# knights-lab/UTree

Measured on AMD Instinct MI355X. Metric: reads classified/sec, 8 GB L2 CTR, 150 bp reads, higher is better.
Workload: dtype u64

## Files before the change

utree_amd/csrc/dev_image.c:

```c
#define _FILE_OFFSET_BITS 64
#define _GNU_SOURCE
#define __HIP_PLATFORM_AMD__ 1
#include <hip/hip_runtime_api.h>
#include <fcntl.h>
#include <math.h>
#include <stddef.h>
#include <stdio.h>
#include <stdlib.h>
#include <string.h>
#include <unistd.h>
#include "ctr_host.h"
#include "dev_image.h"

#define HIPCHK(x) do { hipError_t e_ = (x); if (e_ != hipSuccess) { utree_dev_set_hip_error((int)e_, #x); rc = e_ == hipErrorOutOfMemory ? UTREE_E_NOMEM : UTREE_E_HIP; goto fail; } } while (0)
#define KCHK(x) do { int e_ = (x); if (e_ != 0) { utree_dev_set_hip_error(e_, #x); rc = e_ == (int)hipErrorOutOfMemory ? UTREE_E_NOMEM : UTREE_E_HIP; goto fail; } } while (0)

static __thread char g_hip_msg[256];
void utree_dev_set_hip_error(int err, const char *what) {
    snprintf(g_hip_msg, sizeof g_hip_msg, "%s (%d) in %s", hipGetErrorString((hipError_t)err), err, what);
    if (getenv("UTREE_DEBUG")) fprintf(stderr, "[utree_amd] HIP error: %s\n", g_hip_msg);
}
const char *utree_last_hip_error(void) { return g_hip_msg; }

#include <time.h>
// ... 123 lines not shown
    }
    h->off_coarse = off; off = align_up(off + (uint64_t)UTREE_NUMBINS * ((h->flags & UTREE_F_OFF64) ? 8 : 4), 256);
    h->off_irreg = off; off = align_up(off + (1u << 24) / 8, 256);
    h->off_label_off = off; off = align_up(off + ((uint64_t)h->n_labels + 1) * 4, 256);
    uint64_t blob = 0;
    for (uint32_t i = 0; i < h->n_labels; ++i) blob += (uint64_t)ctr->label_len[i] + 1;
    h->label_blob_bytes = blob;
    h->off_label_blob = off; off = align_up(off + blob + 64, 256);
    h->off_rank2ix = off; off = align_up(off + (uint64_t)h->n_labels * 4, 256);
    h->off_vote = off; off = align_up(off + (uint64_t)h->n_labels * sizeof(utk_vote_rec), 4096);
    h->off_recs = off; off = align_up(off + (h->n_nodes + 8) * h->rec_words * 8, 4096);
    h->total_bytes = off;
}

size_t utree_dev_image_bytes(const utree_ctr *ctr, int fine_bits) {
    if (!ctr) return 0;
    utree_image_header h;
    layout(ctr, (uint32_t)utree_pick_fine_bits(ctr, fine_bits), &h);
    return (size_t)h.total_bytes;
}

static void bind_image(utree_dev *d) {
    char *b = (char *)d->image;
    d->kimg.table = (const uint64_t *)(b + d->hdr.off_table);
    d->kimg.regions = (const uint64_t *)(b + offsetof(utree_image_header, regions));
    d->kimg.mrecs = (const uint64_t *)(b + d->hdr.off_mrecs);
    d->kimg.recs = (const uint64_t *)(b + d->hdr.off_recs);
    d->kimg.coarse = b + d->hdr.off_coarse;
    d->kimg.irreg = (const uint32_t *)(b + d->hdr.off_irreg);
    d->kimg.label_off = (const uint32_t *)(b + d->hdr.off_label_off);
    d->kimg.label_blob = b + d->hdr.off_label_blob;
    d->kimg.rank2ix = (const uint32_t *)(b + d->hdr.off_rank2ix);
    d->kimg.vote_tab = (d->hdr.flags & UTREE_F_VOTE_TABLE) && !getenv("UTREE_VOTE_BYTES") ? (const uint64_t *)(b + d->hdr.off_vote) : NULL;
    d->kimg.n_nodes = d->hdr.n_nodes;
    d->kimg.n_labels = d->hdr.n_labels;
    d->kimg.fine_bits = d->hdr.fine_bits;
    d->kimg.flags = d->hdr.flags;
    d->kimg.W = d->hdr.W; d->kimg.I = d->hdr.I;
    d->kimg.bucket_words = d->hdr.bucket_words;
    {
        const char *e = getenv("UTREE_OVF_SCAN");
        d->kimg.ovf_scan = e && atoi(e) > 0 && atoi(e) <= 1024 ? (uint32_t)atoi(e) : (d->hdr.n_min * 4 > d->hdr.n_nodes ? 16u : 32u);
    }
    d->kimg.irr_n = 0;
    for (int i = 0; i < 4; ++i) d->kimg.irr_p[i] = 0xFFFFFFFFu;
    if (d->hdr.flags & UTREE_F_GENERIC) d->kimg.irr_n = 0xFFFFFFFFu;
    else if (d->hdr.flags & UTREE_F_IRREGULAR) {
        d->kimg.irr_n = 0xFFFFFFFFu;
        uint32_t *bm = d->hdr.n_irregular <= 4 ? (uint32_t *)malloc((1u << 24) / 8) : NULL;
        if (bm && hipMemcpy(bm, d->kimg.irreg, (1u << 24) / 8, hipMemcpyDeviceToHost) == hipSuccess) {
            uint32_t n = 0, p[4] = {0, 0, 0, 0};
            for (uint32_t w = 0; w < (1u << 24) / 32 && n <= 4; ++w)
                for (uint32_t x = bm[w]; x && n <= 4; x &= x - 1) { if (n < 4) p[n] = w * 32 + (uint32_t)__builtin_ctz(x); ++n; }
            if (n <= 4) { d->kimg.irr_n = n; for (uint32_t i = 0; i < n; ++i) d->kimg.irr_p[i] = p[i]; }
        } else (void)hipGetLastError();
        free(bm);
    }
}

static void lanes_ring_init(utree_dev *d);
static int device_ok(int device, int *n_cu) {
    int n = 0;
    if (hipGetDeviceCount(&n) != hipSuccess || device < 0 || device >= n) return UTREE_E_HIP;
    if (hipSetDevice(device) != hipSuccess) return UTREE_E_HIP;
    hipDeviceProp_t p;
    if (hipGetDeviceProperties(&p, device) != hipSuccess) return UTREE_E_HIP;
// ... 613 lines not shown
        if (w.long_blocks) {
            if (e0) HIPCHK(hipEventRecord(e0, st));
            HIPCHK(hipMemsetAsync(w.ltab_rank, 0xFF, (size_t)w.n_long_cap * UTREE_LONG_SLOTS * 4, st));
            HIPCHK(hipMemsetAsync(w.ltab_cnt, 0, (size_t)w.n_long_cap * UTREE_LONG_SLOTS * 4, st));
            HIPCHK(hipMemsetAsync(w.lflag, 0, (size_t)w.n_long_cap * 4, st));
            KCHK(utk_classify_long_pieces(&d->kimg, d_bases, d_off, d_len, do_rc, d_out, &w, d->n_cu, st));
            utk_workspace wl = w;
            wl.long_list = w.long_left;
            wl.long_blocks = w.long_blocks >= 8 ? w.long_blocks / 8 : 1;
            KCHK(utk_classify_long(&d->kimg, d_bases, d_off, d_len, do_rc, d_out, &wl, d->n_cu, st));
            if (e0) { HIPCHK(hipEventRecord(e1, st)); d->recorded[tslot] = 1; }
        }
        KCHK(utk_classify_listed(&d->kimg, d_bases, d_off, d_len, n_reads, max_len, do_rc, d_out, &w, d->n_cu, st));
        if (e0 && !w.long_blocks) { HIPCHK(hipEventRecord(e1, st)); d->recorded[tslot] = 1; }
    } else {
        const int dominant = w.long_blocks ? 2 : (w.mid_reads ? 1 : 0);
        d->last_long = dominant == 2; d->last_mid = dominant == 1; d->last_rc = do_rc; d->last_short_cap = w.short_cap;
        d->last_lanes = 0; d->last_mixed = 0; d->last_pieces = 0;
        if (w.mid_reads) KCHK(utk_route(d_len, n_reads, do_rc, &w, st));
        if (e0 && dominant == 0) HIPCHK(hipEventRecord(e0, st));
        KCHK(utk_classify_short(&d->kimg, d_bases, d_off, d_len, n_reads, do_rc, d_out, &w, d->n_cu, st));
        if (e0 && dominant == 0) { HIPCHK(hipEventRecord(e1, st)); d->recorded[tslot] = 1; }
        if (w.mid_reads) {
            if (e0 && dominant == 1) HIPCHK(hipEventRecord(e0, st));
            KCHK(utk_classify_mid(&d->kimg, d_bases, d_off, d_len, n_reads, do_rc, d_out, &w, d->n_cu, st));
            if (e0 && dominant == 1) { HIPCHK(hipEventRecord(e1, st)); d->recorded[tslot] = 1; }
        }
        if (w.long_blocks) {
            if (e0) HIPCHK(hipEventRecord(e0, st));
            KCHK(utk_classify_long(&d->kimg, d_bases, d_off, d_len, do_rc, d_out, &w, d->n_cu, st));
            if (e0) { HIPCHK(hipEventRecord(e1, st)); d->recorded[tslot] = 1; }
        }
    }
    KCHK(utk_vote(&d->kimg, d_out, &w, n_reads, st));
    if (ring_post(d, &w, lanes ? n_reads : 0, st)) { (void)hipGetLastError(); }
    { ring_lock(d); const unsigned long long pe = d->dev_error; ring_unlock(d);
      if (pe) { rc = UTREE_E_DEVICE; snprintf(g_hip_msg, sizeof g_hip_msg, "an earlier batch's kernels reported error %llu: utree_classify_poll returns (and clears) it", pe); } }
#ifdef UTREE_LANES_TIMERS
    { extern void utk_lanes_phase_dump(void); static int lcalls; if (++lcalls == 6) utk_lanes_phase_dump(); }
#endif
#ifdef UTREE_PHASE_TIMERS
    { extern void utk_phase_dump(void); static int calls; if (++calls == 12) utk_phase_dump(); }
#endif
fail:
    return rc;
}

int utree_lookup_words(utree_dev *d, const uint64_t *d_hi, const uint64_t *d_lo, uint64_t n, uint32_t *d_ix, void *stream) {
    int rc = UTREE_OK;
    if (!d || !d_lo || !d_ix) return UTREE_E_ARG;
    if (d->hdr.W == 16 && !d_hi) return UTREE_E_ARG;
    HIPCHK(hipSetDevice(d->device));
    KCHK(utk_lookup(&d->kimg, d_hi, d_lo, n, d_ix, (hipStream_t)stream));
fail:
    return rc;
}

const char *utree_classify_kernel_name(const utree_dev *dc) {
    if (!dc) return "";
    utree_dev *d = (utree_dev *)dc;
    if (d->last_lanes && d->last_pieces) {
        snprintf(d->kernel_sig, sizeof d->kernel_sig, "classify_lanes_k<%u, %u, 16, %s, 2, %u, %s>", d->hdr.W, d->hdr.I, d->kimg.irr_n ? "true" : "false", d->hdr.bucket_words / 8,
                 utk_lanes_both_strands(&d->kimg, d->last_rc) ? "true" : "false");
        return d->kernel_sig;
    }
    if (d->last_lanes && d->last_mixed) {
        snprintf(d->kernel_sig, sizeof d->kernel_sig, "classify_lanes_mixed_k<%u, %u, %s, %u, %s>", d->hdr.W, d->hdr.I, d->kimg.irr_n ? "true" : "false",
// ... 53 lines not shown
```

utree_amd/csrc/kernels.hip:

```cpp
#include <hip/hip_runtime.h>
#include <stdint.h>
#include <stdio.h>
#include <string.h>
#include "device_common.hpp"
#include "wave_common.hpp"

using namespace utk;

namespace {

#ifdef UTREE_PHASE_TIMERS
__device__ unsigned long long g_phase[16];
struct PhaseT { unsigned long long t, acc[12]; };
#define PH_DECL PhaseT ph_; ph_.t = __builtin_readcyclecounter(); for (int q_ = 0; q_ < 12; ++q_) ph_.acc[q_] = 0;
#define TICKP(ph, i) do { const unsigned long long n_ = __builtin_readcyclecounter(); (ph).acc[i] += n_ - (ph).t; (ph).t = n_; } while (0)
#define TICK(i) TICKP(ph_, i)
#define PH_ARG , PhaseT &ph_
#define PH_PASS , ph_
#define PH_WAITVM asm volatile("s_waitcnt vmcnt(0)" ::: "memory")
#else
#define PH_DECL
#define TICK(i)
#define PH_ARG
#define PH_PASS
#define PH_WAITVM
#endif


constexpr uint32_t KEY_TILE = 128;

struct LaneBits {
    const uint32_t *swl;
    uint32_t sh;
};
__device__ __forceinline__ LaneBits lane_bits(const uint32_t *sw, uint32_t lane) {
    LaneBits b;
    const uint32_t r = lane & 15u;
    b.swl = sw + (lane >> 4) - (r == 0 ? 1u : 0u);
// ... 612 lines not shown
#pragma unroll
        for (int d = 1; d < 64; d <<= 1) { uint32_t t = __shfl_up(inc, d); if (lane >= (uint32_t)d) inc += t; }
        if (lane == 63) s_scan[wv] = inc;
        __syncthreads();
        uint32_t wbase = 0, uix = 0;
        for (uint32_t w = 0; w < LONG_THREADS / 64; ++w) { if (w < wv) wbase += s_scan[w]; uix += s_scan[w]; }
        uint32_t pos = wbase + inc - cnt;
        if (tid == 0) s_base = uix > 1 ? reserve_tally(ws, (unsigned long long)uix) : 0ull;
        __syncthreads();
        const unsigned long long base = s_base;
        for (uint32_t x = lo; x < hi; ++x) {
            uint32_t bits = __hip_atomic_load(&touch[x], __ATOMIC_RELAXED, __HIP_MEMORY_SCOPE_AGENT);
            if (!bits) continue;
            __hip_atomic_store(&touch[x], 0u, __ATOMIC_RELAXED, __HIP_MEMORY_SCOPE_AGENT);
            while (bits) {
                const uint32_t rk = x * 32 + (uint32_t)__builtin_ctz(bits);
                bits &= bits - 1;
                const uint32_t c = __hip_atomic_load(&hist[rk], __ATOMIC_RELAXED, __HIP_MEMORY_SCOPE_AGENT);
                __hip_atomic_store(&hist[rk], 0u, __ATOMIC_RELAXED, __HIP_MEMORY_SCOPE_AGENT);
                if (uix > 1) ws.tally[base + pos] = (uint64_t)rk | ((uint64_t)c << 32);
                else s_single = rk;
                ++pos;
            }
        }
        __syncthreads();
        if (tid == 0) {
            if (uix == 1) store_result(&out[r], im.rank2ix[s_single], -2, F, 1, 0, 0);
            else store_result(&out[r], 0, CUT_PENDING, F, uix, (uint32_t)base, (uint32_t)(base >> 32));
        }
        __syncthreads();
    }
}

__device__ __forceinline__ uint32_t cut_of(uint32_t x) {
    uint32_t c = x - x / 4;
    c += (x >> 1) >= c;
    return c;
}

__device__ __forceinline__ void label16(const char *s, uint32_t p, uint64_t &x, uint64_t &y) {
    typedef unsigned long long u64x2 __attribute__((ext_vector_type(2), aligned(1)));
    const u64x2 v = *(const u64x2 *)(s + p);
    x = v.x; y = v.y;
}

__device__ __forceinline__ uint64_t stop_flags(uint64_t x1, uint64_t x2) {
    const uint64_t semi = x1 ^ 0x3B3B3B3B3B3B3B3Bull, d = x1 ^ x2;
    uint64_t m = (((x1 - 0x0101010101010101ull) & ~x1) | ((semi - 0x0101010101010101ull) & ~semi)) & 0x8080808080808080ull;
    m |= (((d & 0x7F7F7F7F7F7F7F7Full) + 0x7F7F7F7F7F7F7F7Full) | d) & 0x8080808080808080ull;
    return m;
}

__device__ __forceinline__ void pair_scan(const char *s1, const char *s2, uint32_t start, uint32_t &td, uint32_t &a, uint32_t &b, uint32_t &before) {
    uint32_t base = start, prevlast = start ? (uint32_t)(uint8_t)s1[start - 1] : 0u;
    for (;;) {
        uint64_t x1, y1, x2, y2;
        label16(s1, base, x1, y1); label16(s2, base, x2, y2);
        uint64_t m = stop_flags(x1, x2);
        if (!m) { prevlast = (uint32_t)(x1 >> 56); base += 8; x1 = y1; x2 = y2; m = stop_flags(x1, x2); }
        if (m) {
            const uint32_t idx = (uint32_t)(__builtin_ctzll(m) >> 3);
            td = base + idx;
            a = (uint32_t)(x1 >> (8 * idx)) & 0xFFu; b = (uint32_t)(x2 >> (8 * idx)) & 0xFFu;
            before = idx ? ((uint32_t)(x1 >> (8 * idx - 8)) & 0xFFu) : prevlast;
            return;
        }
        prevlast = (uint32_t)(x1 >> 56); base += 8;
    }
}

struct VRec { uint64_t w[4]; };
__device__ __forceinline__ VRec vrec(const uint64_t *vt, uint32_t rank) {
    typedef unsigned long long u64x2 __attribute__((ext_vector_type(2)));
    const u64x2 *p = (const u64x2 *)(vt + (size_t)rank * 4);
    const u64x2 a = p[0], b = p[1];
    VRec v; v.w[0] = a.x; v.w[1] = a.y; v.w[2] = b.x; v.w[3] = b.y;
    return v;
}
__device__ __forceinline__ uint32_t v_pid(const VRec &v, uint32_t t) { return (uint32_t)((t < 4 ? v.w[0] : v.w[1]) >> (16u * (t & 3u))) & 0xFFFFu; }
__device__ __forceinline__ uint32_t v_end(const VRec &v, uint32_t t) { return (uint32_t)(v.w[2] >> (8u * t)) & 0xFFu; }
__device__ __forceinline__ bool v_exists(const VRec &v, uint32_t t) { return ((uint32_t)v.w[3] >> t) & 1u; }
__device__ __forceinline__ bool v_more(const VRec &v, uint32_t t) { return ((uint32_t)v.w[3] >> (8u + t)) & 1u; }
__device__ __forceinline__ bool v_us(const VRec &v, uint32_t t) { return ((uint32_t)v.w[3] >> (16u + t)) & 1u; }
__device__ __forceinline__ uint32_t v_len(const VRec &v) { return (uint32_t)(v.w[3] >> 32) & 0xFFu; }
__device__ __forceinline__ uint32_t v_ix(const VRec &v) { return (uint32_t)(v.w[3] >> 48); }

__device__ __forceinline__ void vote_table(const utk_image &im, utree_result *out_r, const uint64_t *T, uint32_t F, uint32_t uix) {
    const uint64_t *vt = im.vote_tab;
    const char *blob = im.label_blob;
    const uint32_t *loff = im.label_off;
    constexpr uint32_t NONE = 0xFFFFFFFFu;
    uint32_t cutoff = cut_of(F);
    uint32_t st = 0, ed = uix, dv = NONE, t = 0, orun = F, sl, ol;
    uint32_t ix_last, n_last, len_last;
    for (;;) {
        const uint64_t t_st = T[st];
        VRec pv = vrec(vt, (uint32_t)t_st);
        const uint64_t t_ed = ed - 1u == st ? t_st : T[ed - 1u];
        const VRec lv = ed - 1u == st ? pv : vrec(vt, (uint32_t)t_ed);
        {
            const uint64_t d0 = pv.w[0] ^ lv.w[0], d1 = pv.w[1] ^ lv.w[1];
            const uint32_t same = d0 ? (uint32_t)__builtin_ctzll(d0) >> 4 : 4u + (d1 ? (uint32_t)__builtin_ctzll(d1) >> 4 : 4u);
            const uint32_t both = ((uint32_t)(pv.w[3] & lv.w[3]) >> 8) & 0xFFu;
            const uint32_t semis = (uint32_t)__builtin_ctz(~both);
            const uint32_t L = same < semis ? same : semis;
            if (L > t) { dv = v_end(pv, L - 1u); t = L; }
        }
        uint32_t run = (uint32_t)(t_st >> 32), td = dv, c1 = run, rp = (uint32_t)t_st;
        bool td_is_end = false;
        bool stopped = false;
        for (uint32_t z = st + 1; z < ed; ++z) {
            const bool is_last = z == ed - 1u;
            const uint64_t tz = is_last ? t_ed : T[z];
            const uint32_t nz = (uint32_t)(tz >> 32), rc = (uint32_t)tz;
            const VRec cv = is_last ? lv : vrec(vt, rc);
            bool aside = false, stop = false;
            if (t >= 8u || !v_exists(pv, t) || (dv == NONE && v_end(pv, 0) == 0u && !v_more(pv, 0))) aside = true;
            else {
                uint32_t a, b, before;
                bool known = true;
                if (v_exists(cv, t) && v_pid(cv, t) == v_pid(pv, t)) {
                    td = v_end(pv, t); td_is_end = true;
                    a = v_more(pv, t) ? ';' : 0u; b = v_more(cv, t) ? ';' : 0u; before = v_us(pv, t) ? '_' : 'x';
                } else if (v_us(pv, t) || !v_exists(cv, t)) {
                    pair_scan(blob + loff[rp], blob + loff[rc], dv + 1u, td, a, b, before);
                    td_is_end = td == v_end(pv, t);
                } else { a = 'a'; b = 'b'; before = 'x'; known = false; }
                if (a == b) run += nz;
                else if ((!a && b == ';') || ((a == ';' || !a) && before == '_')) aside = true;
                else if (run >= cutoff) {
                    ed = z; stop = true;
                    if (!known) {
                        pair_scan(blob + loff[rp], blob + loff[rc], dv + 1u, td, a, b, before);
                        td_is_end = td == v_end(pv, t);
                    }
                } else { run = nz; st = z; }
            }
            if (aside) {
                run = nz; st = z;
                orun -= c1;
                cutoff = cut_of(orun);
            }
            if (stop) { stopped = true; break; }
            pv = cv; c1 = nz; rp = rc;
        }
        ix_last = stopped ? v_ix(pv) : v_ix(lv);
        n_last = stopped ? c1 : (uint32_t)(t_ed >> 32);
        len_last = stopped ? v_len(pv) : v_len(lv);
        sl = run; ol = orun;
        if (run < cutoff) break;
        if (st + 1 >= ed) {
            if (n_last >= cutoff) dv = 0xFFFFFFFEu;
            break;
        }
        orun = run; cutoff = cut_of(run);
        if (td != dv) { dv = td; if (td_is_end) ++t; }
    }
    int32_t cut;
    if (dv == NONE) cut = -1;
    else if (dv == 0xFFFFFFFEu) cut = -2;
    else cut = (int32_t)(dv < len_last ? dv : len_last);
    store_result(out_r, ix_last, cut, F, uix, sl, ol);
}

#ifdef UTREE_VOTE_WPE8
__attribute__((amdgpu_waves_per_eu(8, 8)))
#endif
__global__ __launch_bounds__(256) void vote_table_k(utk_image im, utree_result *__restrict__ out, utk_workspace ws, uint32_t n_reads) {
#ifndef UTREE_VOTE_UNSORTED
    __shared__ uint32_t s_n[2][4];
    __shared__ uint16_t s_who[256];
    const uint32_t tid = threadIdx.x, wv = tid >> 6, lane = tid & 63u;
    const uint32_t r0 = blockIdx.x * blockDim.x + tid;
    uint32_t cls = 2;
    if (r0 < n_reads) {
        const uint32_t *res = (const uint32_t *)&out[r0];
        const int32_t cut = (int32_t)res[1];
        if (cut == RANK_PENDING) {
            uint32_t *o = (uint32_t *)&out[r0];
            o[0] = im.rank2ix[res[0]]; o[1] = (uint32_t)-2;
        } else if (cut == CUT_PENDING) cls = res[3] == 2u ? 0u : 1u;
    }
    const uint64_t m0 = __builtin_amdgcn_ballot_w64(cls == 0u), m1 = __builtin_amdgcn_ballot_w64(cls == 1u);
    s_who[tid] = 0xFFFFu;
    if (lane == 0) { s_n[0][wv] = (uint32_t)__popcll(m0); s_n[1][wv] = (uint32_t)__popcll(m1); }
    __syncthreads();
    if (cls < 2u) {
        uint32_t before = 0;
        for (uint32_t w = 0; w < wv; ++w) before += s_n[cls][w];
        before += (uint32_t)__popcll((cls ? m1 : m0) & ((1ull << lane) - 1ull));
        s_who[cls ? 255u - before : before] = (uint16_t)tid;
    }
    __syncthreads();
    const uint32_t who = s_who[tid];
    if (who == 0xFFFFu) return;
    const uint32_t r = blockIdx.x * blockDim.x + who;
#else
    const uint32_t r = blockIdx.x * blockDim.x + threadIdx.x;
    if (r >= n_reads) return;
    {
        const uint32_t *res = (const uint32_t *)&out[r];
        if ((int32_t)res[1] == RANK_PENDING) {
            uint32_t *o = (uint32_t *)&out[r];
            o[0] = im.rank2ix[res[0]]; o[1] = (uint32_t)-2;
            return;
        }
        if ((int32_t)res[1] != CUT_PENDING) return;
    }
#endif
    const uint32_t *res = (const uint32_t *)&out[r];
    vote_table(im, &out[r], ws.tally + ((uint64_t)res[4] | ((uint64_t)res[5] << 32)), res[2], res[3]);
}

__global__ __launch_bounds__(256) void vote_k(utk_image im, utree_result *__restrict__ out, utk_workspace ws, uint32_t n_reads) {
    const uint32_t r = blockIdx.x * blockDim.x + threadIdx.x;
    if (r >= n_reads) return;
    const uint32_t *res = (const uint32_t *)&out[r];
    if ((int32_t)res[1] == RANK_PENDING) {
        uint32_t *o = (uint32_t *)&out[r];
        o[0] = im.rank2ix[res[0]]; o[1] = (uint32_t)-2;
        return;
    }
    if ((int32_t)res[1] != CUT_PENDING) return;
    const uint32_t F = res[2], uix = res[3];
    const uint64_t *T = ws.tally + ((uint64_t)res[4] | ((uint64_t)res[5] << 32));
    const char *blob = im.label_blob;
    const uint32_t *loff = im.label_off;
    uint32_t cutoff = cut_of(F);
    uint32_t st = 0, ed = uix, dv = 0xFFFFFFFFu, orun = F, sl, ol;
    for (;;) {
        const uint64_t t_st = T[st];
        {
            const char *sa = blob + loff[(uint32_t)t_st], *sz = blob + loff[(uint32_t)T[ed - 1]];
            uint32_t base = dv + (dv == 0xFFFFFFFFu), q = 0xFFFFFFFFu;
            bool first = dv != 0xFFFFFFFFu;
            for (;;) {
                uint64_t a[2], b[2];
                label16(sa, base, a[0], a[1]); label16(sz, base, b[0], b[1]);
                bool stop = false;
#pragma unroll
                for (int h = 0; h < 2; ++h) {
                    const uint64_t x = a[h], d = a[h] ^ b[h], sx = a[h] ^ 0x3B3B3B3B3B3B3B3Bull;
                    uint64_t end = ((x - 0x0101010101010101ull) & ~x) & 0x8080808080808080ull;
                    end |= (((d & 0x7F7F7F7F7F7F7F7Full) + 0x7F7F7F7F7F7F7F7Full) | d) & 0x8080808080808080ull;
// ... 191 lines not shown
    uint32_t cap = (uint32_t)n_cu * 2u;
    if (blocks > cap) blocks = cap;
    const uint64_t total = do_rc ? 2ull * max_len + 1 : max_len;
    return dispatch_img(im, [&](auto w, auto i, auto exc, auto offt) {
        if (total > SHORT2_CAP)
            classify_short_k<decltype(w)::value, decltype(i)::value, decltype(exc)::value, decltype(offt), MID_CAP, true>
                <<<dim3(blocks), dim3(256), 0, (hipStream_t)stream>>>(*im, d_bases, d_off, d_len, n_reads, do_rc, d_out, *ws);
        else if (do_rc || total > SHORT_CAP)
            classify_short_k<decltype(w)::value, decltype(i)::value, decltype(exc)::value, decltype(offt), SHORT2_CAP, true>
                <<<dim3(blocks), dim3(256), 0, (hipStream_t)stream>>>(*im, d_bases, d_off, d_len, n_reads, do_rc, d_out, *ws);
        else
            classify_short_k<decltype(w)::value, decltype(i)::value, decltype(exc)::value, decltype(offt), SHORT_CAP, true, 0>
                <<<dim3(blocks), dim3(256), 0, (hipStream_t)stream>>>(*im, d_bases, d_off, d_len, n_reads, do_rc, d_out, *ws);
    });
}

int utk_classify_long(const utk_image *im, const uint8_t *d_bases, const uint64_t *d_off, const uint32_t *d_len,
                      int do_rc, utree_result *d_out, const utk_workspace *ws, int n_cu, void *stream) {
    (void)n_cu;
    if (!ws->long_blocks) return 0;
    return dispatch_img_all(im, [&](auto w, auto i, auto exc, auto offt) {
        classify_long_k<decltype(w)::value, decltype(i)::value, decltype(exc)::value, decltype(offt)>
            <<<dim3(ws->long_blocks), dim3(LONG_THREADS), 0, (hipStream_t)stream>>>(*im, d_bases, d_off, d_len, do_rc, d_out, *ws);
    });
}

int utk_vote(const utk_image *im, utree_result *d_out, const utk_workspace *ws, uint32_t n_reads, void *stream) {
    if (!n_reads) return 0;
    if (im->vote_tab) vote_table_k<<<dim3((n_reads + 255) / 256), dim3(256), 0, (hipStream_t)stream>>>(*im, d_out, *ws, n_reads);
    else vote_k<<<dim3((n_reads + 255) / 256), dim3(256), 0, (hipStream_t)stream>>>(*im, d_out, *ws, n_reads);
    return (int)hipGetLastError();
}

int utk_lookup(const utk_image *im, const uint64_t *d_hi, const uint64_t *d_lo, uint64_t n, uint32_t *d_ix, void *stream) {
    if (!n) return 0;
    uint64_t blocks = (n + 255) / 256;
    if (blocks > 8192) blocks = 8192;
    return dispatch_img_all(im, [&](auto w, auto i, auto exc, auto offt) {
        lookup_k<decltype(w)::value, decltype(i)::value, decltype(exc)::value, decltype(offt)>
            <<<dim3((unsigned)blocks), dim3(256), 0, (hipStream_t)stream>>>(*im, d_hi, d_lo, n, d_ix);
    });
}

#ifdef UTREE_PHASE_TIMERS
void utk_phase_dump(void) {
    unsigned long long h[16];
    static const char *nm[12] = {"grab", "next read's len/off + fetch issue", "minimizers", "round: address (LDS chain) + load issue", "round: wait for the bucket",
                                 "round: scan", "round: hit compaction", "stage next read (waits for its bytes)", "tally + result", "after windows", "", ""};
    if (hipDeviceSynchronize() != hipSuccess || hipMemcpyFromSymbol(h, HIP_SYMBOL(g_phase), sizeof h) != hipSuccess) return;
    unsigned long long tot = 0;
    for (int q = 0; q < 12; ++q) tot += h[q];
    fprintf(stderr, "[phase timers] %llu waves, %.3g cycles per wave\n", h[12], h[12] ? (double)tot / h[12] : 0.0);
    for (int q = 0; q < 10; ++q) fprintf(stderr, "  %-45s %5.1f %%\n", nm[q], tot ? 100.0 * h[q] / tot : 0.0);
    memset(h, 0, sizeof h);
    (void)hipMemcpyToSymbol(HIP_SYMBOL(g_phase), h, sizeof h);
}
#endif

int utk_model_counts(const utk_image *im, const uint8_t *d_bases, const uint64_t *d_off, const uint32_t *d_len, uint32_t n_reads,
                     int do_rc, unsigned long long *d_counts, void *stream) {
    if (!n_reads) return 0;
    uint32_t blocks = (n_reads + 3) / 4;
    if (blocks > 4096) blocks = 4096;
    return dispatch_wi(im->W, im->I, [&](auto w, auto i) {
        model_k<decltype(w)::value, decltype(i)::value><<<dim3(blocks), dim3(256), 0, (hipStream_t)stream>>>(*im, d_bases, d_off, d_len, n_reads,
                                                                                                      do_rc, d_counts);
// ... 19 lines not shown
```

utree_amd/csrc/lanes_core.hpp:

```cpp
#pragma once
#include <hip/hip_runtime.h>
#include <stdint.h>
#include <stdio.h>
#include <string.h>
#include "device_common.hpp"
#include "wave_common.hpp"

using namespace utk;

#ifndef UTREE_LANES_WAVES
#define UTREE_LANES_WAVES 4
#endif
#ifndef UTREE_LANES_WPS
#define UTREE_LANES_WPS 3
#endif
#ifndef UTREE_LANES_WPS64
#define UTREE_LANES_WPS64 3
#endif
#ifndef UTREE_LANES_TSLOTS
#define UTREE_LANES_TSLOTS 12
#endif

namespace {

#ifdef UTREE_LANES_TIMERS
__device__ unsigned long long g_lphase[8];
#define LT_DECL unsigned long long lt_t = __builtin_readcyclecounter(), lt_acc[6] = {0, 0, 0, 0, 0, 0};
#define LT(i) do { const unsigned long long n_ = __builtin_readcyclecounter(); lt_acc[i] += n_ - lt_t; lt_t = n_; } while (0)
#else
#define LT_DECL
#define LT(i)
#endif

constexpr int LANES_WAVES = UTREE_LANES_WAVES;
constexpr uint32_t LCAP = UTREE_LANES_CAP;
constexpr uint32_t NWORD = LCAP / 16;
static_assert(LCAP % 32 == 0, "slot geometry");
static_assert(LCAP + 16 + 48 <= 256, "positions are 8-bit fields of a run record");
template <int W> struct Geo {
// ... 719 lines not shown
        const bool live = have && !exc;
        const uint32_t *tq = tab + (lane < RPW ? lane : 0u);
        uint32_t nu = 0, F = 0;
        if (live) {
#pragma unroll
            for (uint32_t i = 0; i < TSR; ++i) { const uint32_t e = tq[i * RPW]; if (e != T_EMPTY) { ++nu; F += e & CMASK; } }
        }
        const uint32_t first_rank = tq[0] >> CB;
        const uint32_t maxnu = uni32(wave_max_u32(nu));
        const uint32_t need = nu >= 2u ? nu : 0u;
        uint32_t incl = need;
#pragma unroll
        for (int dd = 1; dd < 64; dd <<= 1) { const uint32_t t = __shfl_up(incl, dd); if (lane >= (uint32_t)dd) incl += t; }
        const uint32_t total = uni32((uint32_t)__shfl(incl, 63));
        if (total > chunk_left) {
            unsigned long long nb = 0;
            if (lane == 0) {
                nb = atomicAdd(&ws.cursors[0], (unsigned long long)UTREE_TALLY_CHUNK);
                if (nb + UTREE_TALLY_CHUNK > ws.tally_cap) { ws.cursors[UTREE_CUR_ERROR] = UTREE_DEVERR_TALLY_CAP; nb = 0; }
            }
            chunk_base = uni64(nb);
            chunk_left = UTREE_TALLY_CHUNK;
        }
        const unsigned long long my_base = chunk_base + (incl - need);
        chunk_base += total; chunk_left -= total;
        if (maxnu >= 2u) {
            for (uint32_t i = 0; i < maxnu; ++i) {
                const uint32_t e = tq[i * RPW];
                uint32_t place = 0;
                for (uint32_t j = 0; j < maxnu; ++j) { const uint32_t x = tq[j * RPW]; place += (j < nu && (x >> CB) < (e >> CB)) ? 1u : 0u; }
                if (need && i < nu) ws.tally[my_base + place] = (uint64_t)(e >> CB) | ((uint64_t)(e & CMASK) << 32);
            }
        }
        if (live) {
            if (F == 0) store_result(&out[r], 0, -2, 0, 0, 0, 0);
            else if (nu == 1) store_result(&out[r], first_rank, RANK_PENDING, F, 1, 0, 0);
            else store_result(&out[r], 0, CUT_PENDING, F, nu, (uint32_t)my_base, (uint32_t)(my_base >> 32));
        }
        wave_lds_fence();
        LT(4);
    }
#ifdef UTREE_LANES_TIMERS
    if (lane == 0) { for (int q = 0; q < 6; ++q) atomicAdd(&g_lphase[q], lt_acc[q]); atomicAdd(&g_lphase[7], 1ull); }
#endif
}

#define LANES_PROLOGUE(W_) \
    using G_ = Geo<W_>; \
    __shared__ uint32_t s_stream[LANES_WAVES][64 * G_::STRIDE]; \
    __shared__ uint32_t s_runs[LANES_WAVES][G_::RUNS]; \
    __shared__ uint32_t s_tab[LANES_WAVES][64 * TSLOTS]; \
    __shared__ uint32_t s_full[LANES_WAVES][2]; \
    __shared__ uint32_t s_pref[LANES_WAVES][64]; \
    __shared__ uint64_t s_ost[LANES_WAVES][64]; \
    __shared__ uint64_t s_reg[256]; \
    for (uint32_t x = threadIdx.x; x < 256; x += blockDim.x) s_reg[x] = im.regions[x]; \
    const uint32_t wv = uni32(threadIdx.x >> 6); \
    { uint32_t *sl_ = s_stream[wv] + lane_id() * G_::STRIDE + G_::FRONT; \
      _Pragma("unroll") for (uint32_t i = 1; i <= G_::FRONT; ++i) sl_[-(int)i] = 0;       \
      sl_[NWORD] = 0; sl_[NWORD + 1] = 0; } \
    __syncthreads();
#define LANES_LDS s_stream[wv], s_runs[wv], s_tab[wv], s_full[wv], s_pref[wv], s_ost[wv], s_reg, wv

template <int W, int I, int SEGS, bool IRR, int MODE, int NL, bool BS>
__global__ __launch_bounds__(LANES_WAVES * 64, W == 16 ? UTREE_LANES_WPS64 : UTREE_LANES_WPS)
void classify_lanes_k(utk_image im, const uint8_t *__restrict__ bases, const uint64_t *__restrict__ off, const uint32_t *__restrict__ len,
                      uint32_t n_reads, int do_rc, utree_result *__restrict__ out, utk_workspace ws, uint32_t cls) {
    LANES_PROLOGUE(W)
    lanes_body<W, I, SEGS, IRR, MODE, NL, BS>(im, bases, off, len, n_reads, do_rc, out, ws, cls, LANES_LDS);
}

// ... 40 lines not shown
```

utree_amd/csrc/utree_internal.h:

```cpp
#ifndef UTREE_INTERNAL_H
#define UTREE_INTERNAL_H
#include <stddef.h>
#include <stdint.h>
#include "../../include/utree_amd.h"

#ifdef __cplusplus
extern "C" {
#endif

#define UTREE_NUMBINS ((1u << 24) + 1u)
#define UTREE_INVALID 0xFFFFFFFFu
#define UTREE_IMG_MAGIC 0x31474d4945525455ull
#define UTREE_IMG_HEADER_BYTES 4096u
#define UTREE_IMG_VERSION 14u
#ifndef UTREE_CANON_MODE
#define UTREE_CANON_MODE 1
#endif
#define UTREE_REGION_NB_BITS 25
#define UTREE_REGION_SUB_BITS 9
#define UTREE_REGION_BASE_SHIFT (UTREE_REGION_NB_BITS + UTREE_REGION_SUB_BITS)
#define UTREE_MIN_MARGIN(W_) ((W_) == 16 ? 2u : 0u)
#define UTREE_TALLY_CHUNK 8192u
#define UTREE_CUR_LONG 32
#define UTREE_CUR_MID 16
// ... 20 lines not shown
#define UTREE_F_IRREGULAR 1u
#define UTREE_F_GENERIC   2u
#define UTREE_F_OFF64     4u
#define UTREE_F_VOTE_TABLE 16u
#define UTREE_F_STRAND_VIEWS 32u
#define UTREE_F_DIRECT 64u
#define UTREE_F_OVF_CHAINS 128u
#define UTREE_F_INVALID_RANKS 8u

typedef struct {
    uint64_t magic;
    uint32_t version, W, I, k;
    uint32_t fine_bits, rec_words, n_labels, flags;
    uint64_t n_nodes;
    uint64_t n_slots;
    uint64_t n_min;
    uint64_t off_table, off_mrecs, off_recs, off_coarse, off_irreg, off_label_off, off_label_blob, off_rank2ix;
    uint64_t label_blob_bytes;
    uint64_t n_irregular;
    uint64_t total_bytes;
    uint64_t off_vote;
    uint32_t bucket_words, pad0;
    uint64_t regions[256];
} utree_image_header;

typedef struct {
    uint16_t pid[8];
    uint8_t tok_end[8];
    uint8_t exists, more, us, n_tok;
    uint8_t len, pad;
    uint16_t ix;
} utk_vote_rec;

typedef struct {
    const uint64_t *table;
    const uint64_t *regions;
    const uint64_t *mrecs;
    const uint64_t *recs;
    const void *coarse;
    const uint32_t *irreg;
    const uint32_t *label_off;
    const char *label_blob;
    const uint32_t *rank2ix;
    const uint64_t *vote_tab;
    uint64_t n_nodes;
    uint32_t n_labels, fine_bits, flags, W, I;
    uint32_t bucket_words;
    uint32_t ovf_scan;
    uint32_t irr_n, irr_p[4];
} utk_image;

static inline uint32_t utree_rec_words(uint32_t W, uint32_t I) { return (W == 16 ? 2u : 1u) * (I == 4 ? 2u : 1u); }

int utk_repack(uint32_t W, uint32_t I, const void *d_raw, uint64_t count, const uint32_t *d_ix2rank,
               uint32_t n_labels, uint64_t *d_recs_at_first, unsigned long long *d_invalid, void *stream);
int utk_widen_binix(const void *d_raw_binix, uint32_t width, int off64, void *d_coarse, void *stream);
int utk_validate(uint32_t W, uint32_t I, int off64, const void *d_coarse, const uint64_t *d_recs, uint64_t n_nodes,
                 uint32_t *d_irreg, unsigned long long *d_counters, void *stream);
int utk_build_min(uint32_t W, uint32_t I, int off64, const void *d_coarse, const uint64_t *d_recs, uint64_t c0, uint64_t m, uint64_t dup_cap,
                  const uint64_t *d_regions, const uint64_t *h_regions, uint64_t n_buckets, uint32_t bucket_words, uint64_t *d_table, uint64_t *d_mrecs,
                  uint32_t *d_irreg, unsigned long long *d_overflow, uint64_t *n_min, int *views, void *stream);
int utk_build_direct(uint32_t I, int off64, int generic, const void *d_coarse, const uint64_t *d_recs, uint64_t n_nodes, uint64_t c0, uint64_t m,
                     const uint32_t *d_irreg, uint64_t n_irregular, void *d_table, void *stream);
int utk_compact_overflow(uint32_t W, uint32_t I, uint64_t *d_table, uint64_t n_buckets, uint32_t bucket_words, uint64_t *d_mrecs, uint64_t *n_kept, int *chains, void *stream);
int utk_compress_chunk(uint32_t W, uint32_t I, const void *d_in, uint64_t first, uint64_t count, unsigned long long *d_first,
                       void *d_out, void *stream);
int utk_fill_recs_pad(uint64_t *d_recs_end, uint32_t words, void *stream);

typedef struct {
    unsigned long long *cursors;
    uint64_t *tally;
    uint64_t tally_cap;
    uint32_t *long_list;
    uint32_t *mid_list;
    uint32_t *hist;
    uint32_t *touch;
    uint32_t long_blocks, mid_reads;
    uint32_t short_cap;
    uint32_t mid_limit;
    uint64_t *pieces;
    uint32_t *ltab_rank, *ltab_cnt;
    uint32_t *lflag;
    uint32_t *long_left;
    uint32_t n_long_cap;
    uint64_t n_pieces_cap;
    uint32_t *cls_list;
    uint32_t cls_stride;
    uint64_t ltally_base;
} utk_workspace;

int utk_classify_short(const utk_image *im, const uint8_t *d_bases, const uint64_t *d_off, const uint32_t *d_len,
                       uint32_t n_reads, int do_rc, utree_result *d_out, const utk_workspace *ws, int n_cu,
                       void *stream);
int utk_lanes_ok(const utk_image *im, uint32_t max_len, int do_rc);
int utk_lanes_segs(const utk_image *im, uint32_t max_len);
int utk_lanes_image_ok(const utk_image *im);
int utk_lanes_both_strands(const utk_image *im, int do_rc);
int utk_classify_long_pieces(const utk_image *im, const uint8_t *d_bases, const uint64_t *d_off, const uint32_t *d_len, int do_rc,
                             utree_result *d_out, const utk_workspace *ws, int n_cu, void *stream);
int utk_classify_lanes(const utk_image *im, const uint8_t *d_bases, const uint64_t *d_off, const uint32_t *d_len, uint32_t n_reads,
                       uint32_t max_len, int do_rc, utree_result *d_out, const utk_workspace *ws, int n_cu, void *stream);
int utk_classify_lanes_mixed(const utk_image *im, const uint8_t *d_bases, const uint64_t *d_off, const uint32_t *d_len, uint32_t n_reads,
                             uint32_t max_len, int do_rc, utree_result *d_out, const utk_workspace *ws, int n_cu, void *stream);
uint32_t utk_lanes_max_len(const utk_image *im);
int utk_route(const uint32_t *d_len, uint32_t n_reads, int do_rc, const utk_workspace *ws, void *stream);
int utk_classify_mid(const utk_image *im, const uint8_t *d_bases, const uint64_t *d_off, const uint32_t *d_len,
                     uint32_t n_reads, int do_rc, utree_result *d_out, const utk_workspace *ws, int n_cu, void *stream);
int utk_classify_listed(const utk_image *im, const uint8_t *d_bases, const uint64_t *d_off, const uint32_t *d_len,
                        uint32_t n_reads, uint32_t max_len, int do_rc, utree_result *d_out, const utk_workspace *ws, int n_cu, void *stream);
int utk_classify_long(const utk_image *im, const uint8_t *d_bases, const uint64_t *d_off, const uint32_t *d_len,
                      int do_rc, utree_result *d_out, const utk_workspace *ws, int n_cu, void *stream);
int utk_vote(const utk_image *im, utree_result *d_out, const utk_workspace *ws, uint32_t n_reads, void *stream);
int utk_lookup(const utk_image *im, const uint64_t *d_hi, const uint64_t *d_lo, uint64_t n, uint32_t *d_ix,
               void *stream);
typedef struct {
    unsigned long long *cursors;
    uint32_t *nh;
    uint64_t *hoff;
    uint32_t *hits;
    uint64_t hits_cap;
    uint32_t *lvl[3];
    uint32_t nlvl[3];
    uint32_t *hist;
    uint32_t hist_waves;
    uint32_t *state;
    uint32_t state_cap;
    uint32_t step;
    uint32_t slack, tolerance;
} utk_rank_ws;

int utk_rank_hits(const utk_image *im, const uint8_t *d_bases, const uint64_t *d_off, const uint32_t *d_len,
                  uint32_t n_reads, int do_rc, const utk_rank_ws *ws, int n_cu, void *stream);
int utk_rank_levels(const utk_rank_ws *ws, uint32_t n_reads, void *stream);
int utk_rank_vote(const utk_image *im, utree_result *d_out, uint32_t n_reads, const utk_rank_ws *ws, int n_cu,
                  void *stream);
int utk_rank_state(uint32_t n_reads, const utk_rank_ws *ws, void *stream);

const char *utk_classify_short_name(const utk_image *im, uint32_t short_cap, int mid, int do_rc, char *buf, size_t cap);
const char *utk_classify_long_name(const utk_image *im, char *buf, size_t cap);
int utk_model_counts(const utk_image *im, const uint8_t *d_bases, const uint64_t *d_off, const uint32_t *d_len, uint32_t n_reads,
                     int do_rc, unsigned long long *d_counts, void *stream);

#ifdef __cplusplus
}
#endif
// ... 2 lines not shown
```

Measured before the change: 2.428 billion.

## Fuse table-based voting into lanes classify kernel with wave-level sorting

After: 2.389 billion, median of 6. -1.6%, worse.

```diff
diff --git a/utree_amd/csrc/dev_image.c b/utree_amd/csrc/dev_image.c
--- a/utree_amd/csrc/dev_image.c
+++ b/utree_amd/csrc/dev_image.c
@@ -179,6 +179,10 @@
     d->kimg.label_blob = b + d->hdr.off_label_blob;
     d->kimg.rank2ix = (const uint32_t *)(b + d->hdr.off_rank2ix);
     d->kimg.vote_tab = (d->hdr.flags & UTREE_F_VOTE_TABLE) && !getenv("UTREE_VOTE_BYTES") ? (const uint64_t *)(b + d->hdr.off_vote) : NULL;
+    {
+        const char *e = getenv("UTREE_LANE_VOTE");
+        d->kimg.lane_vote = UTREE_LANES_VOTE && d->kimg.vote_tab && !(e && e[0] == '0');
+    }
     d->kimg.n_nodes = d->hdr.n_nodes;
     d->kimg.n_labels = d->hdr.n_labels;
     d->kimg.fine_bits = d->hdr.fine_bits;
@@ -858,7 +862,8 @@
             if (e0) { HIPCHK(hipEventRecord(e1, st)); d->recorded[tslot] = 1; }
         }
     }
-    KCHK(utk_vote(&d->kimg, d_out, &w, n_reads, st));
+    if (lanes && d->kimg.lane_vote && !w.long_blocks) KCHK(utk_vote_listed(&d->kimg, d_out, &w, d->n_cu, st));
+    else KCHK(utk_vote(&d->kimg, d_out, &w, n_reads, st));
     if (ring_post(d, &w, lanes ? n_reads : 0, st)) { (void)hipGetLastError(); }
     { ring_lock(d); const unsigned long long pe = d->dev_error; ring_unlock(d);
       if (pe) { rc = UTREE_E_DEVICE; snprintf(g_hip_msg, sizeof g_hip_msg, "an earlier batch's kernels reported error %llu: utree_classify_poll returns (and clears) it", pe); } }
diff --git a/utree_amd/csrc/kernels.hip b/utree_amd/csrc/kernels.hip
--- a/utree_amd/csrc/kernels.hip
+++ b/utree_amd/csrc/kernels.hip
@@ -4,6 +4,7 @@
 #include <string.h>
 #include "device_common.hpp"
 #include "wave_common.hpp"
+#include "vote_table.hpp"
 
 using namespace utk;
 
@@ -682,136 +683,6 @@
     }
 }
 
-__device__ __forceinline__ uint32_t cut_of(uint32_t x) {
-    uint32_t c = x - x / 4;
-    c += (x >> 1) >= c;
-    return c;
-}
-
-__device__ __forceinline__ void label16(const char *s, uint32_t p, uint64_t &x, uint64_t &y) {
-    typedef unsigned long long u64x2 __attribute__((ext_vector_type(2), aligned(1)));
-    const u64x2 v = *(const u64x2 *)(s + p);
-    x = v.x; y = v.y;
-}
-
-__device__ __forceinline__ uint64_t stop_flags(uint64_t x1, uint64_t x2) {
-    const uint64_t semi = x1 ^ 0x3B3B3B3B3B3B3B3Bull, d = x1 ^ x2;
-    uint64_t m = (((x1 - 0x0101010101010101ull) & ~x1) | ((semi - 0x0101010101010101ull) & ~semi)) & 0x8080808080808080ull;
-    m |= (((d & 0x7F7F7F7F7F7F7F7Full) + 0x7F7F7F7F7F7F7F7Full) | d) & 0x8080808080808080ull;
-    return m;
-}
-
-__device__ __forceinline__ void pair_scan(const char *s1, const char *s2, uint32_t start, uint32_t &td, uint32_t &a, uint32_t &b, uint32_t &before) {
-    uint32_t base = start, prevlast = start ? (uint32_t)(uint8_t)s1[start - 1] : 0u;
-    for (;;) {
-        uint64_t x1, y1, x2, y2;
-        label16(s1, base, x1, y1); label16(s2, base, x2, y2);
-        uint64_t m = stop_flags(x1, x2);
-        if (!m) { prevlast = (uint32_t)(x1 >> 56); base += 8; x1 = y1; x2 = y2; m = stop_flags(x1, x2); }
-        if (m) {
-            const uint32_t idx = (uint32_t)(__builtin_ctzll(m) >> 3);
-            td = base + idx;
-            a = (uint32_t)(x1 >> (8 * idx)) & 0xFFu; b = (uint32_t)(x2 >> (8 * idx)) & 0xFFu;
-            before = idx ? ((uint32_t)(x1 >> (8 * idx - 8)) & 0xFFu) : prevlast;
-            return;
-        }
-        prevlast = (uint32_t)(x1 >> 56); base += 8;
-    }
-}
-
-struct VRec { uint64_t w[4]; };
-__device__ __forceinline__ VRec vrec(const uint64_t *vt, uint32_t rank) {
-    typedef unsigned long long u64x2 __attribute__((ext_vector_type(2)));
-    const u64x2 *p = (const u64x2 *)(vt + (size_t)rank * 4);
-    const u64x2 a = p[0], b = p[1];
-    VRec v; v.w[0] = a.x; v.w[1] = a.y; v.w[2] = b.x; v.w[3] = b.y;
-    return v;
-}
-__device__ __forceinline__ uint32_t v_pid(const VRec &v, uint32_t t) { return (uint32_t)((t < 4 ? v.w[0] : v.w[1]) >> (16u * (t & 3u))) & 0xFFFFu; }
-__device__ __forceinline__ uint32_t v_end(const VRec &v, uint32_t t) { return (uint32_t)(v.w[2] >> (8u * t)) & 0xFFu; }
-__device__ __forceinline__ bool v_exists(const VRec &v, uint32_t t) { return ((uint32_t)v.w[3] >> t) & 1u; }
-__device__ __forceinline__ bool v_more(const VRec &v, uint32_t t) { return ((uint32_t)v.w[3] >> (8u + t)) & 1u; }
-__device__ __forceinline__ bool v_us(const VRec &v, uint32_t t) { return ((uint32_t)v.w[3] >> (16u + t)) & 1u; }
-__device__ __forceinline__ uint32_t v_len(const VRec &v) { return (uint32_t)(v.w[3] >> 32) & 0xFFu; }
-__device__ __forceinline__ uint32_t v_ix(const VRec &v) { return (uint32_t)(v.w[3] >> 48); }
-
-__device__ __forceinline__ void vote_table(const utk_image &im, utree_result *out_r, const uint64_t *T, uint32_t F, uint32_t uix) {
-    const uint64_t *vt = im.vote_tab;
-    const char *blob = im.label_blob;
-    const uint32_t *loff = im.label_off;
-    constexpr uint32_t NONE = 0xFFFFFFFFu;
-    uint32_t cutoff = cut_of(F);
-    uint32_t st = 0, ed = uix, dv = NONE, t = 0, orun = F, sl, ol;
-    uint32_t ix_last, n_last, len_last;
-    for (;;) {
-        const uint64_t t_st = T[st];
-        VRec pv = vrec(vt, (uint32_t)t_st);
-        const uint64_t t_ed = ed - 1u == st ? t_st : T[ed - 1u];
-        const VRec lv = ed - 1u == st ? pv : vrec(vt, (uint32_t)t_ed);
-        {
-            const uint64_t d0 = pv.w[0] ^ lv.w[0], d1 = pv.w[1] ^ lv.w[1];
-            const uint32_t same = d0 ? (uint32_t)__builtin_ctzll(d0) >> 4 : 4u + (d1 ? (uint32_t)__builtin_ctzll(d1) >> 4 : 4u);
-            const uint32_t both = ((uint32_t)(pv.w[3] & lv.w[3]) >> 8) & 0xFFu;
-            const uint32_t semis = (uint32_t)__builtin_ctz(~both);
-            const uint32_t L = same < semis ? same : semis;
-            if (L > t) { dv = v_end(pv, L - 1u); t = L; }
-        }
-        uint32_t run = (uint32_t)(t_st >> 32), td = dv, c1 = run, rp = (uint32_t)t_st;
-        bool td_is_end = false;
-        bool stopped = false;
-        for (uint32_t z = st + 1; z < ed; ++z) {
-            const bool is_last = z == ed - 1u;
-            const uint64_t tz = is_last ? t_ed : T[z];
-            const uint32_t nz = (uint32_t)(tz >> 32), rc = (uint32_t)tz;
-            const VRec cv = is_last ? lv : vrec(vt, rc);
-            bool aside = false, stop = false;
-            if (t >= 8u || !v_exists(pv, t) || (dv == NONE && v_end(pv, 0) == 0u && !v_more(pv, 0))) aside = true;
-            else {
-                uint32_t a, b, before;
-                bool known = true;
-                if (v_exists(cv, t) && v_pid(cv, t) == v_pid(pv, t)) {
-                    td = v_end(pv, t); td_is_end = true;
-                    a = v_more(pv, t) ? ';' : 0u; b = v_more(cv, t) ? ';' : 0u; before = v_us(pv, t) ? '_' : 'x';
-                } else if (v_us(pv, t) || !v_exists(cv, t)) {
-                    pair_scan(blob + loff[rp], blob + loff[rc], dv + 1u, td, a, b, before);
-                    td_is_end = td == v_end(pv, t);
-                } else { a = 'a'; b = 'b'; before = 'x'; known = false; }
-                if (a == b) run += nz;
-                else if ((!a && b == ';') || ((a == ';' || !a) && before == '_')) aside = true;
-                else if (run >= cutoff) {
-                    ed = z; stop = true;
-                    if (!known) {
-                        pair_scan(blob + loff[rp], blob + loff[rc], dv + 1u, td, a, b, before);
-                        td_is_end = td == v_end(pv, t);
-                    }
-                } else { run = nz; st = z; }
-            }
-            if (aside) {
-                run = nz; st = z;
-                orun -= c1;
-                cutoff = cut_of(orun);
-            }
-            if (stop) { stopped = true; break; }
-            pv = cv; c1 = nz; rp = rc;
-        }
-        ix_last = stopped ? v_ix(pv) : v_ix(lv);
-        n_last = stopped ? c1 : (uint32_t)(t_ed >> 32);
-        len_last = stopped ? v_len(pv) : v_len(lv);
-        sl = run; ol = orun;
-        if (run < cutoff) break;
-        if (st + 1 >= ed) {
-            if (n_last >= cutoff) dv = 0xFFFFFFFEu;
-            break;
-        }
-        orun = run; cutoff = cut_of(run);
-        if (td != dv) { dv = td; if (td_is_end) ++t; }
-    }
-    int32_t cut;
-    if (dv == NONE) cut = -1;
-    else if (dv == 0xFFFFFFFEu) cut = -2;
-    else cut = (int32_t)(dv < len_last ? dv : len_last);
-    store_result(out_r, ix_last, cut, F, uix, sl, ol);
-}
 
 #ifdef UTREE_VOTE_WPE8
 __attribute__((amdgpu_waves_per_eu(8, 8)))
@@ -859,7 +730,24 @@
     }
 #endif
     const uint32_t *res = (const uint32_t *)&out[r];
-    vote_table(im, &out[r], ws.tally + ((uint64_t)res[4] | ((uint64_t)res[5] << 32)), res[2], res[3]);
+    const VoteOut v = vote_table(im, ws.tally + ((uint64_t)res[4] | ((uint64_t)res[5] << 32)), res[2], res[3]);
+    store_result(&out[r], v.ix, v.cut, res[2], res[3], v.sl, v.ol);
+}
+
+__global__ __launch_bounds__(256) void vote_listed_k(utk_image im, utree_result *__restrict__ out, utk_workspace ws) {
+    const uint32_t n = (uint32_t)ws.cursors[UTREE_CUR_MID];
+    for (uint32_t i = blockIdx.x * blockDim.x + threadIdx.x; i < n; i += gridDim.x * blockDim.x) {
+        const uint32_t r = ws.mid_list[i];
+        const uint32_t *res = (const uint32_t *)&out[r];
+        const int32_t cut = (int32_t)res[1];
+        if (cut == RANK_PENDING) {
+            uint32_t *o = (uint32_t *)&out[r];
+            o[0] = im.rank2ix[res[0]]; o[1] = (uint32_t)-2;
+        } else if (cut == CUT_PENDING) {
+            const VoteOut v = vote_table(im, ws.tally + ((uint64_t)res[4] | ((uint64_t)res[5] << 32)), res[2], res[3]);
+            store_result(&out[r], v.ix, v.cut, res[2], res[3], v.sl, v.ol);
+        }
+    }
 }
 
 __global__ __launch_bounds__(256) void vote_k(utk_image im, utree_result *__restrict__ out, utk_workspace ws, uint32_t n_reads) {
@@ -1117,6 +1005,11 @@
     return (int)hipGetLastError();
 }
 
+int utk_vote_listed(const utk_image *im, utree_result *d_out, const utk_workspace *ws, int n_cu, void *stream) {
+    vote_listed_k<<<dim3((unsigned)(n_cu > 0 ? n_cu : 1)), dim3(256), 0, (hipStream_t)stream>>>(*im, d_out, *ws);
+    return (int)hipGetLastError();
+}
+
 int utk_lookup(const utk_image *im, const uint64_t *d_hi, const uint64_t *d_lo, uint64_t n, uint32_t *d_ix, void *stream) {
     if (!n) return 0;
     uint64_t blocks = (n + 255) / 256;
diff --git a/utree_amd/csrc/lanes_core.hpp b/utree_amd/csrc/lanes_core.hpp
--- a/utree_amd/csrc/lanes_core.hpp
+++ b/utree_amd/csrc/lanes_core.hpp
@@ -5,6 +5,7 @@
 #include <string.h>
 #include "device_common.hpp"
 #include "wave_common.hpp"
+#include "vote_table.hpp"
 
 using namespace utk;
 
@@ -790,11 +791,36 @@
                 if (need && i < nu) ws.tally[my_base + place] = (uint64_t)(e >> CB) | ((uint64_t)(e & CMASK) << 32);
             }
         }
+        const bool vote = UTREE_LANES_VOTE && im.lane_vote != 0u;
         if (live) {
             if (F == 0) store_result(&out[r], 0, -2, 0, 0, 0, 0);
-            else if (nu == 1) store_result(&out[r], first_rank, RANK_PENDING, F, 1, 0, 0);
-            else store_result(&out[r], 0, CUT_PENDING, F, nu, (uint32_t)my_base, (uint32_t)(my_base >> 32));
-        }
+            else if (nu == 1) {
+                if (vote) store_result(&out[r], im.rank2ix[first_rank], -2, F, 1, 0, 0);
+                else store_result(&out[r], first_rank, RANK_PENDING, F, 1, 0, 0);
+            } else if (!vote) store_result(&out[r], 0, CUT_PENDING, F, nu, (uint32_t)my_base, (uint32_t)(my_base >> 32));
+        }
+#if UTREE_LANES_VOTE
+        if (vote && maxnu >= 2u) {
+            const bool multi = live && nu >= 2u;
+            uint32_t vr = r, vF = F, vnu = multi ? nu : 0u;
+            unsigned long long vbase = my_base;
+#ifndef UTREE_LANE_VOTE_UNSORTED
+            const uint64_t m2 = ballot64(multi && nu == 2u), mm = ballot64(multi && nu > 2u), mo = ~(m2 | mm);
+            const uint32_t dest = multi ? (nu == 2u ? lanes_below(m2) : 63u - lanes_below(mm)) : (uint32_t)__popcll(m2) + lanes_below(mo);
+            const int da = (int)(dest << 2);
+            vr = (uint32_t)__builtin_amdgcn_ds_permute(da, (int)vr);
+            vF = (uint32_t)__builtin_amdgcn_ds_permute(da, (int)vF);
+            vnu = (uint32_t)__builtin_amdgcn_ds_permute(da, (int)vnu);
+            vbase = (unsigned long long)(uint32_t)__builtin_amdgcn_ds_permute(da, (int)(uint32_t)vbase)
+                  | ((unsigned long long)(uint32_t)__builtin_amdgcn_ds_permute(da, (int)(uint32_t)(vbase >> 32)) << 32);
+            __builtin_amdgcn_fence(__ATOMIC_ACQ_REL, "workgroup");
+#endif
+            if (vnu >= 2u) {
+                const VoteOut v = vote_table(im, ws.tally + vbase, vF, vnu);
+                store_result(&out[vr], v.ix, v.cut, vF, vnu, v.sl, v.ol);
+            }
+        }
+#endif
         wave_lds_fence();
         LT(4);
     }
diff --git a/utree_amd/csrc/utree_internal.h b/utree_amd/csrc/utree_internal.h
--- a/utree_amd/csrc/utree_internal.h
+++ b/utree_amd/csrc/utree_internal.h
@@ -76,6 +76,10 @@
     uint16_t ix;
 } utk_vote_rec;
 
+#ifndef UTREE_LANES_VOTE
+#define UTREE_LANES_VOTE 0
+#endif
+
 typedef struct {
     const uint64_t *table;
     const uint64_t *regions;
@@ -92,6 +96,7 @@
     uint32_t bucket_words;
     uint32_t ovf_scan;
     uint32_t irr_n, irr_p[4];
+    uint32_t lane_vote;
 } utk_image;
 
 static inline uint32_t utree_rec_words(uint32_t W, uint32_t I) { return (W == 16 ? 2u : 1u) * (I == 4 ? 2u : 1u); }
@@ -155,6 +160,7 @@
 int utk_classify_long(const utk_image *im, const uint8_t *d_bases, const uint64_t *d_off, const uint32_t *d_len,
                       int do_rc, utree_result *d_out, const utk_workspace *ws, int n_cu, void *stream);
 int utk_vote(const utk_image *im, utree_result *d_out, const utk_workspace *ws, uint32_t n_reads, void *stream);
+int utk_vote_listed(const utk_image *im, utree_result *d_out, const utk_workspace *ws, int n_cu, void *stream);
 int utk_lookup(const utk_image *im, const uint64_t *d_hi, const uint64_t *d_lo, uint64_t n, uint32_t *d_ix,
                void *stream);
 typedef struct {
diff --git a/utree_amd/csrc/vote_table.hpp b/utree_amd/csrc/vote_table.hpp
--- /dev/null
+++ b/utree_amd/csrc/vote_table.hpp
@@ -0,0 +1,141 @@
+#pragma once
+#include <hip/hip_runtime.h>
+#include <stdint.h>
+#include "utree_internal.h"
+
+namespace {
+
+struct VoteOut { uint32_t ix; int32_t cut; uint32_t sl, ol; };
+
+__device__ __forceinline__ uint32_t cut_of(uint32_t x) {
+    uint32_t c = x - x / 4;
+    c += (x >> 1) >= c;
+    return c;
+}
+
+__device__ __forceinline__ void label16(const char *s, uint32_t p, uint64_t &x, uint64_t &y) {
+    typedef unsigned long long u64x2 __attribute__((ext_vector_type(2), aligned(1)));
+    const u64x2 v = *(const u64x2 *)(s + p);
+    x = v.x; y = v.y;
+}
+
+__device__ __forceinline__ uint64_t stop_flags(uint64_t x1, uint64_t x2) {
+    const uint64_t semi = x1 ^ 0x3B3B3B3B3B3B3B3Bull, d = x1 ^ x2;
+    uint64_t m = (((x1 - 0x0101010101010101ull) & ~x1) | ((semi - 0x0101010101010101ull) & ~semi)) & 0x8080808080808080ull;
+    m |= (((d & 0x7F7F7F7F7F7F7F7Full) + 0x7F7F7F7F7F7F7F7Full) | d) & 0x8080808080808080ull;
+    return m;
+}
+
+__device__ __forceinline__ void pair_scan(const char *s1, const char *s2, uint32_t start, uint32_t &td, uint32_t &a, uint32_t &b, uint32_t &before) {
+    uint32_t base = start, prevlast = start ? (uint32_t)(uint8_t)s1[start - 1] : 0u;
+    for (;;) {
+        uint64_t x1, y1, x2, y2;
+        label16(s1, base, x1, y1); label16(s2, base, x2, y2);
+        uint64_t m = stop_flags(x1, x2);
+        if (!m) { prevlast = (uint32_t)(x1 >> 56); base += 8; x1 = y1; x2 = y2; m = stop_flags(x1, x2); }
+        if (m) {
+            const uint32_t idx = (uint32_t)(__builtin_ctzll(m) >> 3);
+            td = base + idx;
+            a = (uint32_t)(x1 >> (8 * idx)) & 0xFFu; b = (uint32_t)(x2 >> (8 * idx)) & 0xFFu;
+            before = idx ? ((uint32_t)(x1 >> (8 * idx - 8)) & 0xFFu) : prevlast;
+            return;
+        }
+        prevlast = (uint32_t)(x1 >> 56); base += 8;
+    }
+}
+
+struct VRec { uint64_t w[4]; };
+__device__ __forceinline__ VRec vrec(const uint64_t *vt, uint32_t rank) {
+    typedef unsigned long long u64x2 __attribute__((ext_vector_type(2)));
+    const u64x2 *p = (const u64x2 *)(vt + (size_t)rank * 4);
+    const u64x2 a = p[0], b = p[1];
+    VRec v; v.w[0] = a.x; v.w[1] = a.y; v.w[2] = b.x; v.w[3] = b.y;
+    return v;
+}
+__device__ __forceinline__ uint32_t v_pid(const VRec &v, uint32_t t) { return (uint32_t)((t < 4 ? v.w[0] : v.w[1]) >> (16u * (t & 3u))) & 0xFFFFu; }
+__device__ __forceinline__ uint32_t v_end(const VRec &v, uint32_t t) { return (uint32_t)(v.w[2] >> (8u * t)) & 0xFFu; }
+__device__ __forceinline__ bool v_exists(const VRec &v, uint32_t t) { return ((uint32_t)v.w[3] >> t) & 1u; }
+__device__ __forceinline__ bool v_more(const VRec &v, uint32_t t) { return ((uint32_t)v.w[3] >> (8u + t)) & 1u; }
+__device__ __forceinline__ bool v_us(const VRec &v, uint32_t t) { return ((uint32_t)v.w[3] >> (16u + t)) & 1u; }
+__device__ __forceinline__ uint32_t v_len(const VRec &v) { return (uint32_t)(v.w[3] >> 32) & 0xFFu; }
+__device__ __forceinline__ uint32_t v_ix(const VRec &v) { return (uint32_t)(v.w[3] >> 48); }
+
+__device__ __forceinline__ VoteOut vote_table(const utk_image &im, const uint64_t *T, uint32_t F, uint32_t uix) {
+    const uint64_t *vt = im.vote_tab;
+    const char *blob = im.label_blob;
+    const uint32_t *loff = im.label_off;
+    constexpr uint32_t NONE = 0xFFFFFFFFu;
+    uint32_t cutoff = cut_of(F);
+    uint32_t st = 0, ed = uix, dv = NONE, t = 0, orun = F, sl, ol;
+    uint32_t ix_last, n_last, len_last;
+    for (;;) {
+        const uint64_t t_st = T[st];
+        VRec pv = vrec(vt, (uint32_t)t_st);
+        const uint64_t t_ed = ed - 1u == st ? t_st : T[ed - 1u];
+        const VRec lv = ed - 1u == st ? pv : vrec(vt, (uint32_t)t_ed);
+        {
+            const uint64_t d0 = pv.w[0] ^ lv.w[0], d1 = pv.w[1] ^ lv.w[1];
+            const uint32_t same = d0 ? (uint32_t)__builtin_ctzll(d0) >> 4 : 4u + (d1 ? (uint32_t)__builtin_ctzll(d1) >> 4 : 4u);
+            const uint32_t both = ((uint32_t)(pv.w[3] & lv.w[3]) >> 8) & 0xFFu;
+            const uint32_t semis = (uint32_t)__builtin_ctz(~both);
+            const uint32_t L = same < semis ? same : semis;
+            if (L > t) { dv = v_end(pv, L - 1u); t = L; }
+        }
+        uint32_t run = (uint32_t)(t_st >> 32), td = dv, c1 = run, rp = (uint32_t)t_st;
+        bool td_is_end = false;
+        bool stopped = false;
+        for (uint32_t z = st + 1; z < ed; ++z) {
+            const bool is_last = z == ed - 1u;
+            const uint64_t tz = is_last ? t_ed : T[z];
+            const uint32_t nz = (uint32_t)(tz >> 32), rc = (uint32_t)tz;
+            const VRec cv = is_last ? lv : vrec(vt, rc);
+            bool aside = false, stop = false;
+            if (t >= 8u || !v_exists(pv, t) || (dv == NONE && v_end(pv, 0) == 0u && !v_more(pv, 0))) aside = true;
+            else {
+                uint32_t a, b, before;
+                bool known = true;
+                if (v_exists(cv, t) && v_pid(cv, t) == v_pid(pv, t)) {
+                    td = v_end(pv, t); td_is_end = true;
+                    a = v_more(pv, t) ? ';' : 0u; b = v_more(cv, t) ? ';' : 0u; before = v_us(pv, t) ? '_' : 'x';
+                } else if (v_us(pv, t) || !v_exists(cv, t)) {
+                    pair_scan(blob + loff[rp], blob + loff[rc], dv + 1u, td, a, b, before);
+                    td_is_end = td == v_end(pv, t);
+                } else { a = 'a'; b = 'b'; before = 'x'; known = false; }
+                if (a == b) run += nz;
+                else if ((!a && b == ';') || ((a == ';' || !a) && before == '_')) aside = true;
+                else if (run >= cutoff) {
+                    ed = z; stop = true;
+                    if (!known) {
+                        pair_scan(blob + loff[rp], blob + loff[rc], dv + 1u, td, a, b, before);
+                        td_is_end = td == v_end(pv, t);
+                    }
+                } else { run = nz; st = z; }
+            }
+            if (aside) {
+                run = nz; st = z;
+                orun -= c1;
+                cutoff = cut_of(orun);
+            }
+            if (stop) { stopped = true; break; }
+            pv = cv; c1 = nz; rp = rc;
+        }
+        ix_last = stopped ? v_ix(pv) : v_ix(lv);
+        n_last = stopped ? c1 : (uint32_t)(t_ed >> 32);
+        len_last = stopped ? v_len(pv) : v_len(lv);
+        sl = run; ol = orun;
+        if (run < cutoff) break;
+        if (st + 1 >= ed) {
+            if (n_last >= cutoff) dv = 0xFFFFFFFEu;
+            break;
+        }
+        orun = run; cutoff = cut_of(run);
+        if (td != dv) { dv = td; if (td_is_end) ++t; }
+    }
+    int32_t cut;
+    if (dv == NONE) cut = -1;
+    else if (dv == 0xFFFFFFFEu) cut = -2;
+    else cut = (int32_t)(dv < len_last ? dv : len_last);
+    return VoteOut{ix_last, cut, sl, ol};
+}
+
+}
```
